# vishnutez/dps-ttc

Hardware: AMD Instinct MI355X
Metric: particles×denoise-steps/sec @256×256 N=64; x0_hat rel-L2 vs ref (higher is better)
Workload: dtype f32; 1 GPU; FFHQ-shaped 256x256 Gaussian deblur (sigma=3.0, k=61), 'ps' scale 0.3, one global best-of-N select at the end, N=64 particles (64 per GPU), t cycling 999->0; operator=gaussian_blur, step=dps, particles_per_gpu=64, global_particles=64, image=3x256x256, chains_per_gpu=3, x0_hat_store=False, semantic_stand_in=False

## Files before the change

dps_ttc_amd/csrc/api.hip:

```cpp
#include <cmath>
#include <cstring>
#include <new>
#include <algorithm>
#include <vector>

#include "common.h"

using namespace dpsx;

namespace dpsx {
static thread_local char g_hip_err[256] = "";
void set_last_hip_error(hipError_t e)
{
    snprintf(g_hip_err, sizeof(g_hip_err), "%s: %s", hipGetErrorName(e), hipGetErrorString(e));
}
}

#pragma GCC visibility push(default)
extern "C" {

int dpsx_abi_version(void) { return DPSX_ABI_VERSION; }

const char *dpsx_strerror(int code)
{
// ... 325 lines not shown
    }
    return DPSX_EUNSUPPORTED;
}

int dpsx_residual_norm_f32(const float *y, int64_t y_n, const float *ax, float *r, float *norm, int64_t n,
                           int64_t m, void *workspace, int64_t workspace_bytes, void *stream)
{
    if (!y || !ax || !norm || n < 0 || m < 0 || !rows_ok(y_n, n)) return DPSX_EINVAL;
    if (n == 0) return DPSX_OK;
    const int parts = (int)std::min<int64_t>(256, std::max<int64_t>(1, (m + 4095) / 4096));
    if (!workspace || workspace_bytes < n * parts * 4) return DPSX_EWORKSPACE;
    float *partials = static_cast<float *>(workspace);
    hipStream_t s = (hipStream_t)stream;
    int rc = residual_partials(y, y_n, ax, r, partials, n, m, parts, s);
    if (rc != DPSX_OK) return rc;
    return finalize_norm(partials, parts, norm, n, s);
}

int dpsx_norm_bwd_f32(const float *r, const float *norm, const float *g_norm, int power, float *g_ax, int64_t n,
                      int64_t m, void *stream)
{
    if (!r || !norm || !g_norm || !g_ax || n < 0 || m < 0 || (power != 1 && power != 2)) return DPSX_EINVAL;
    return norm_bwd(r, norm, g_norm, power, g_ax, n, m, (hipStream_t)stream);
}

int64_t dpsx_step_resid_bytes(const dpsx_op *op, int64_t n, int64_t c, int64_t h, int64_t w)
{
    if (!op) return DPSX_EINVAL;
    const int64_t m = meas_elems(op, c, h, w);
    if (m < 0) return DPSX_EINVAL;
    switch (op->kind) {
    case OP_MASK: return 256;
    case OP_PHASE: return phase_step_resid_bytes(op, n * c);
    default: return align256(n * m * 4);
    }
}

static bool mask_fused_ok(const dpsx_op *op, int64_t c, int64_t h, int64_t w,
                          std::initializer_list<const void *> ptrs)
{
    return (h * w) % 4 == 0 && aligned16(op->mask.mask) && vec_ok(c * h * w, ptrs);
}

int dpsx_step_draws_in_kernel(const dpsx_op *op, int64_t c, int64_t h, int64_t w)
{
    if (!op || c < 1 || h < 1 || w < 1) return 0;
    switch (op->kind) {
    case OP_IDENT: return 1;
    case OP_MASK: return (h * w) % 4 == 0 && (c * h * w) % 4 == 0;
    case OP_SEP:
    case OP_TAPS: return blur_step_draws_in_kernel(op, h, w) ? 1 : 0;
    case OP_RESIZE: return h == op->resize->in_h && w == op->resize->in_w && resize_step_draws_in_kernel(op) ? 1 : 0;
    default: return 0;
    }
}

static int step_fwd_impl(dpsx_op *op, const float *x_t, const float *model_out, const float *noise, const dpsx_rng *rng,
                         const float *y, int64_t y_n, float *x0_hat, float *sample, uint8_t *inside, void *resid,
                         float *norm, int64_t n, int64_t c, int64_t h, int64_t w, const dpsx_coefs *coefs_host,
                         void *workspace, int64_t workspace_bytes, void *stream)
{
    int rc = check_geom(op, n, c, h, w);
    if (rc != DPSX_OK) return rc;
    RngK rk{};
    if (rng) {
        if ((rc = to_rngk(rng, n, rk)) != DPSX_OK) return rc;
        if (!dpsx_step_draws_in_kernel(op, c, h, w)) return DPSX_EUNSUPPORTED;
    }
    if (!x_t || !model_out || !y || !sample || !inside || !resid || !coefs_host) return DPSX_EINVAL;
    if (!x0_hat && op && op->kind != OP_SEP && op->kind != OP_TAPS && op->kind != OP_RESIZE &&
        !(op->kind == OP_PHASE && phase_is_spectral(op)))
        return DPSX_EINVAL;
    if ((coefs_host->add_noise & 1) && !noise && !rng) return DPSX_EINVAL;
    if (!rows_ok(y_n, n)) return DPSX_EINVAL;
    if (n == 0) return DPSX_OK;
    Ws ws;
    if ((rc = carve(op, workspace, workspace_bytes, n, c, h, w, ws)) != DPSX_OK) return rc;
    hipStream_t s = (hipStream_t)stream;
    const Coefs k = to_coefs(coefs_host);
    const int64_t chw = c * h * w;
    StepFwdArgs a{x_t, model_out, noise, y, y_n, x0_hat, sample, inside, static_cast<float *>(resid),
                  ws.partials, n, c, h, w, k};
    a.y_div = row_div(y_n, n);
    a.mask_div = row_div(op->mask.rows, n);
    a.use_rng = rng != nullptr;
    a.rng = rk;
    const int parts = step_parts(op, c, h, w);
    bool tail_done = false;
    if (norm && op->d_counters && n <= kTailMaxParticles && op->kind != OP_PHASE) {
        a.tail.counters = op->d_counters;
        a.tail.partials = ws.partials;
        a.tail.parts = parts;
        a.tail.out = norm;
        tail_done = true;
    }
    switch (op->kind) {
    case OP_SEP:
    case OP_TAPS: rc = blur_step_fwd(op, a, s); break;
    case OP_RESIZE: rc = resize_step_fwd(op, a, s); break;
    case OP_MASK:
        if (!mask_fused_ok(op, c, h, w, {x_t, model_out, noise, y, x0_hat, sample}) ||
            !aligned4(inside))
            return DPSX_EUNSUPPORTED;
        rc = mask_step_fwd(op, a, parts, s);
        break;
    case OP_IDENT:
        rc = posterior_fwd(x_t, model_out, noise, a.use_rng, rk, x0_hat, sample, inside, n, chw, k, s);
        if (rc != DPSX_OK) return rc;
        rc = residual_partials(y, y_n, x0_hat, static_cast<float *>(resid), ws.partials, n, chw, parts, s, 0, nullptr, 0, 1,
                               a.tail);
        break;
    case OP_PHASE:
        rc = phase_step_fwd(op, a, static_cast<float *>(resid), s);
        break;
    default: return DPSX_EUNSUPPORTED;
    }
    if (rc != DPSX_OK) {
        if (tail_done)
            (void)hipMemsetAsync(op->d_counters, 0, kNormCounterBytes, s);
        return rc;
    }
    return (norm && !tail_done) ? finalize_norm(ws.partials, parts, norm, n, s) : DPSX_OK;
}

int dpsx_step_fwd_f32(dpsx_op *op, const float *x_t, const float *model_out, const float *noise, const float *y,
                      int64_t y_n, float *x0_hat, float *sample, uint8_t *inside, void *resid, float *norm,
                      int64_t n, int64_t c, int64_t h, int64_t w, const dpsx_coefs *coefs_host, void *workspace,
                      int64_t workspace_bytes, void *stream)
{
    return step_fwd_impl(op, x_t, model_out, noise, nullptr, y, y_n, x0_hat, sample, inside, resid, norm, n, c, h, w,
                         coefs_host, workspace, workspace_bytes, stream);
}

int dpsx_step_fwd_rng_f32(dpsx_op *op, const float *x_t, const float *model_out, const dpsx_rng *rng_host,
                          const float *y, int64_t y_n, float *x0_hat, float *sample, uint8_t *inside, void *resid,
                          float *norm, int64_t n, int64_t c, int64_t h, int64_t w, const dpsx_coefs *coefs_host,
                          void *workspace, int64_t workspace_bytes, void *stream)
{
    if (!rng_host) return DPSX_EINVAL;
    return step_fwd_impl(op, x_t, model_out, nullptr, rng_host, y, y_n, x0_hat, sample, inside, resid, norm, n, c, h, w,
                         coefs_host, workspace, workspace_bytes, stream);
}

int dpsx_step_bwd_f32(dpsx_op *op, const void *resid, const float *norm, float *norm_out, const uint8_t *inside,
                      const float *x0_hat, const float *y, int64_t y_n, float scale, int power,
                      float *g_model_out, int64_t n, int64_t c, int64_t h, int64_t w,
                      const dpsx_coefs *coefs_host, void *workspace, int64_t workspace_bytes, void *stream)
{
    return dpsx_step_bwd_extra_f32(op, resid, norm, norm_out, inside, x0_hat, y, y_n, scale, power, nullptr,
                                   g_model_out, n, c, h, w, coefs_host, workspace, workspace_bytes, stream);
}

int dpsx_step_bwd_extra_f32(dpsx_op *op, const void *resid, const float *norm, float *norm_out,
                            const uint8_t *inside, const float *x0_hat, const float *y, int64_t y_n, float scale,
                            int power, const float *g_x0_extra, float *g_model_out, int64_t n, int64_t c, int64_t h,
                            int64_t w, const dpsx_coefs *coefs_host, void *workspace, int64_t workspace_bytes,
                            void *stream)
{
    int rc = check_geom(op, n, c, h, w);
    if (rc != DPSX_OK) return rc;
    if (!resid || !inside || !g_model_out || !coefs_host || (power != 1 && power != 2)) return DPSX_EINVAL;
    if (!norm && !norm_out) return DPSX_EINVAL;
    if (y && !rows_ok(y_n, n)) return DPSX_EINVAL;
    if (n == 0) return DPSX_OK;
    Ws ws;
    if ((rc = carve(op, workspace, workspace_bytes, n, c, h, w, ws)) != DPSX_OK) return rc;
    hipStream_t s = (hipStream_t)stream;
    const Coefs k = to_coefs(coefs_host);
    const int64_t chw = c * h * w;
    const int parts = step_parts(op, c, h, w);
    if (op->kind == OP_IDENT || op->kind == OP_PHASE) {
        if (!norm && !(op->kind == OP_PHASE && phase_norm_in_bwd(op))) {
            if ((rc = finalize_norm(ws.partials, parts, norm_out, n, s)) != DPSX_OK) return rc;
            norm = norm_out;
        }
    }
    StepBwdArgs b{static_cast<const float *>(resid), norm, ws.partials, parts, norm_out, inside, x0_hat, y, y_n,
                  scale, power, g_model_out, n, c, h, w, k, g_x0_extra};
    b.y_div = row_div(y_n, n);
    b.mask_div = row_div(op->mask.rows, n);
    switch (op->kind) {
    case OP_SEP:
    case OP_TAPS: return blur_step_bwd(op, b, static_cast<float *>(ws.priv), ws.priv_bytes, s);
    case OP_RESIZE: return resize_step_bwd(op, b, s);
    case OP_MASK:
        if (!x0_hat || !y || !rows_ok(y_n, n)) return DPSX_EINVAL;
        if (!mask_fused_ok(op, c, h, w, {x0_hat, y, g_model_out}) || !aligned4(inside))
            return DPSX_EUNSUPPORTED;
        return mask_step_bwd(op, b, s);
    case OP_IDENT:
        return clamp_scale_to_eps(static_cast<const float *>(resid), norm, inside, scale, power, g_model_out, n,
                                  chw, k, s, g_x0_extra);
    case OP_PHASE:
        if (phase_vec4_ok(op) && vec_ok(h, {g_model_out, g_x0_extra}) && aligned4(inside))
            return phase_step_bwd_fused(op, const_cast<float *>(static_cast<const float *>(resid)), b, s);
        if (phase_is_spectral(op)) return DPSX_EUNSUPPORTED;
        rc = phase_step_bwd(op, const_cast<float *>(static_cast<const float *>(resid)), ws.img, n * c, s);
        if (rc != DPSX_OK) return rc;
        return clamp_scale_to_eps(ws.img, norm, inside, scale, power, g_model_out, n, chw, k, s, g_x0_extra);
    }
    return DPSX_EUNSUPPORTED;
}

int dpsx_step_update_f32(const float *sample, const float *g_model_out, const float *g_unet, float *x_next,
                         int64_t n, int64_t chw, const dpsx_coefs *coefs_host, void *stream)
{
    if (!sample || !g_model_out || !x_next || !coefs_host || n < 0 || chw < 0) return DPSX_EINVAL;
    if (coefs_host->b == 0.0f) return DPSX_EINVAL;
    return step_update(sample, g_model_out, g_unet, x_next, n, chw, to_coefs(coefs_host), (hipStream_t)stream);
}

int dpsx_corr_slots(int64_t chw) { return chw < 0 ? DPSX_EINVAL : cg_slots(chw); }

// ... 593 lines not shown
```

dps_ttc_amd/csrc/blur.hip:

```cpp
#include <algorithm>
#include <cmath>
#include <cstdlib>
#include <new>
#include <type_traits>

#include "common.h"

namespace dpsx {

constexpr int TH = 64, TW = 64, NT = 256;
constexpr size_t kScratchBytes = 1024;

struct BlurArgs {
    const float *x;
    float *out;
    const float *x_t, *model_out, *noise;
    float *x0_hat, *sample;
    uint8_t *inside_w;
    const float *y;
    unsigned y_div;
    float *partials;
    const float *norm_in;
    const float *norm_partials;
    int norm_parts;
    float *norm_out;
    const uint8_t *inside_r;
    const float *g_extra;
    float *g_model_out;
    float scale;
    int power;
    int c, h, w, tiles_x, tiles_y, planes;
    Coefs k;
    const TapRun *runs;
    int nrun[4];
    int nhlo[4], nhhi[4];
    int dbg;
    int src_h, src_w, src_off;
    int l1;
    NormTail tail;
    RngK rng;
};

__device__ __forceinline__ bool block_to_tile(const BlurArgs &a, int &plane, int &ty, int &tx)
{
    const int tiles = a.tiles_x * a.tiles_y;
    const int b = blockIdx.x;
    const int xcd = b & 7, k = b >> 3;
    plane = (k / tiles) * 8 + xcd;
    const int t = k % tiles;
    ty = t / a.tiles_x;
    tx = t % a.tiles_x;
    return plane < a.planes;
}

__device__ __forceinline__ int clampi(int v, int lo, int hi) { return v < lo ? lo : (v > hi ? hi : v); }

template <bool POST, bool REFLECT, bool VEC>
__device__ __forceinline__ void load_region(float *s_in, const int SW, const int RH, const int RW,
                                            const int gy0, const int gx0, const int h0, const int w0,
                                            const BlurArgs &a, const int plane, const int tid = threadIdx.x)
{
    const int h = REFLECT ? a.h : a.src_h, w = REFLECT ? a.w : a.src_w, off = REFLECT ? 0 : a.src_off;
    const int64_t hw = (int64_t)h * w;
    const int n = plane / a.c, ch = plane % a.c;
    const float *src = nullptr, *eps = nullptr, *vv = nullptr, *zz = nullptr;
    if constexpr (POST) {
        src = a.x_t + (int64_t)plane * hw;
        eps = a.model_out + ((int64_t)n * 2 * a.c + ch) * hw;
        vv = eps + (int64_t)a.c * hw;
        zz = a.noise + (int64_t)plane * hw;
    } else {
        src = a.x + (int64_t)plane * hw;
    }
// ... 1093 lines not shown

static inline unsigned grid_blocks(const BlurArgs &a)
{
    const int groups = (a.planes + 7) / 8;
    return (unsigned)(groups * 8 * a.tiles_x * a.tiles_y);
}

int64_t blur_parts_per_particle(const dpsx_op *, int64_t c, int64_t h, int64_t w)
{
    return c * ((h + TH - 1) / TH) * ((w + TW - 1) / TW);
}

template <auto Kernel, class... Args>
static int launch(const BlurArgs &a, size_t lds, hipStream_t s, const Args &...args)
{
    return launch_lds<Kernel>(grid_blocks(a), NT, lds, s, a, args...);
}

template <class F> static int with_r4(int r4, F &&f)
{
    switch (r4) {
    case 1: return f(std::integral_constant<int, 1>{});
    case 2: return f(std::integral_constant<int, 2>{});
    case 3: return f(std::integral_constant<int, 3>{});
    case 4: return f(std::integral_constant<int, 4>{});
    case 5: return f(std::integral_constant<int, 5>{});
    case 6: return f(std::integral_constant<int, 6>{});
    case 7: return f(std::integral_constant<int, 7>{});
    case 8: return f(std::integral_constant<int, 8>{});
    }
    return DPSX_EUNSUPPORTED;
}

template <bool POST, bool RESID, bool RNG = false>
static int dispatch_sep_fwd(const BlurTables &b, const BlurArgs &a, hipStream_t s)
{
    return with_r4(b.radius4 / 4, [&](auto r4) {
        constexpr int R4 = decltype(r4)::value;
        return launch<k_blur_sep_fwd<R4, POST, RESID, RNG>>(a, sep_lds_bytes(4 * R4), s, b.sep);
    });
}

template <int R4, bool EPI>
static int launch_sep_adj(const BlurArgs &a, const SepTaps &t, int reach, hipStream_t s)
{
    const size_t lds = sep_lds_bytes(4 * R4, a.h % TH == 0 && a.w % TW == 0 && a.tiles_x >= 2 && a.tiles_y >= 2);
    if constexpr (EPI) {
        if (a.g_extra) return launch<k_blur_sep_adj<R4, true, true>>(a, lds, s, t, reach);
    }
    return launch<k_blur_sep_adj<R4, EPI, false>>(a, lds, s, t, reach);
}

template <int R4, bool EPI>
static int launch_sep_adj_sym(const BlurArgs &a, const SepTaps &t, hipStream_t s)
{
    const size_t lds = sep_lds_bytes(4 * R4, true);
    if constexpr (EPI) {
        if (a.g_extra) return launch<k_blur_sep_adj_sym<R4, true, true>>(a, lds, s, t);
    }
    return launch<k_blur_sep_adj_sym<R4, EPI, false>>(a, lds, s, t);
}

static bool sep_adj_sym_ok(const BlurTables &b, const BlurArgs &a)
{
    static const char *force = getenv("DPSX_SEP_ADJ");
    if (force && force[0] == 'f') return false;
    const int rr = b.radius4;
    if (a.h % TH != 0 || a.w % TW != 0 || a.tiles_x < 2 || a.tiles_y < 2 || rr + 1 >= a.h || rr + 1 >= a.w) return false;
    for (int i = 0; i < rr; ++i)
        if (b.sep.h[i] != b.sep.h[2 * rr - i] || b.sep.v[i] != b.sep.v[2 * rr - i]) return false;
    return true;
}

template <bool EPI>
static int dispatch_sep_adj(const BlurTables &b, const BlurArgs &a, hipStream_t s)
{
    const int rr = b.radius4;
    const bool sym = sep_adj_sym_ok(b, a);
    SepTaps f{};
    if (!sym)
        for (int i = 0; i <= 2 * rr; ++i) {
            f.h[i] = b.sep.h[2 * rr - i];
            f.v[i] = b.sep.v[2 * rr - i];
        }
    return with_r4(rr / 4, [&](auto r4) {
        constexpr int R4 = decltype(r4)::value;
        return sym ? launch_sep_adj_sym<R4, EPI>(a, b.sep, s) : launch_sep_adj<R4, EPI>(a, f, b.reach, s);
    });
}

// ... 132 lines not shown
int blur_forward(const dpsx_op *op, const float *x, float *y, int64_t planes, int64_t h, int64_t w, hipStream_t s)
{
    if (!geometry_ok(op, h, w)) return DPSX_EINVAL;
    if (planes == 0) return DPSX_OK;
    BlurArgs a{};
    a.x = x; a.out = y;
    fill_geometry(a, planes, 1, h, w);
    const bool vec = blur_vec(h, w, {x, y});
    return op->kind == OP_SEP && vec ? dispatch_sep_fwd<false, false>(op->blur->t, a, s)
                                     : launch_taps_fwd<false, false>(*op->blur, a, vec, s);
}

int blur_adjoint(const dpsx_op *op, const float *u, float *g, int64_t planes, int64_t h, int64_t w, float *scratch,
                 int64_t scratch_bytes, hipStream_t s)
{
    if (!geometry_ok(op, h, w)) return DPSX_EINVAL;
    if (planes == 0) return DPSX_OK;
    BlurArgs a{};
    a.x = u; a.out = g;
    fill_geometry(a, planes, 1, h, w);
    const bool vec = blur_vec(h, w, {u, g});
    return op->kind == OP_SEP && vec ? dispatch_sep_adj<false>(op->blur->t, a, s)
                                     : launch_taps_adj<false>(*op->blur, a, vec, scratch, scratch_bytes, s);
}

bool blur_step_draws_in_kernel(const dpsx_op *op, int64_t h, int64_t w)
{
    if (!geometry_ok(op, h, w) || h % TH != 0 || w % TW != 0) return false;
    const BlurTables &b = op->blur->t;
    if (op->kind == OP_SEP) return b.radius4 < h && b.radius4 < w && b.radius4 / 4 >= 1 && b.radius4 / 4 <= 8;
    return std::max(b.halo_t, b.halo_b) < h && std::max(b.halo_l, b.halo_r) < w;
}

int blur_step_fwd(const dpsx_op *op, const StepFwdArgs &f, hipStream_t s)
{
    if (!geometry_ok(op, f.h, f.w)) return DPSX_EINVAL;
    if (f.n == 0) return DPSX_OK;
    BlurArgs a{};
    a.x_t = f.x_t; a.model_out = f.model_out; a.noise = f.noise;
    a.x0_hat = f.x0_hat; a.sample = f.sample; a.inside_w = f.inside;
    a.y = f.y; a.y_div = f.y_div; a.out = f.resid; a.partials = f.partials;
    a.k = f.k;
    fill_geometry(a, f.n * f.c, f.c, f.h, f.w);
    a.tail = f.tail;
    a.tail.blocks_per_particle = a.c * a.tiles_x * a.tiles_y;
    const bool vec = blur_vec(f.h, f.w, {f.x_t, f.model_out, f.noise, f.x0_hat, f.sample, f.y, f.resid}) && aligned4(f.inside);
    if (f.use_rng) {
        if (!vec || !blur_step_draws_in_kernel(op, f.h, f.w)) return DPSX_EUNSUPPORTED;
        a.rng = f.rng;
        return op->kind == OP_SEP ? dispatch_sep_fwd<true, true, true>(op->blur->t, a, s)
                                  : launch_taps_fwd<true, true, true>(*op->blur, a, true, s);
    }
    return op->kind == OP_SEP && vec ? dispatch_sep_fwd<true, true>(op->blur->t, a, s)
                                     : launch_taps_fwd<true, true>(*op->blur, a, vec, s);
}

int blur_step_bwd(const dpsx_op *op, const StepBwdArgs &b, float *scratch, int64_t scratch_bytes, hipStream_t s)
{
    if (!geometry_ok(op, b.h, b.w)) return DPSX_EINVAL;
    if (b.n == 0) return DPSX_OK;
    BlurArgs a{};
    a.x = b.resid;
    a.norm_in = b.norm; a.norm_partials = b.partials; a.norm_parts = b.parts; a.norm_out = b.norm_out;
    a.inside_r = b.inside; a.g_extra = b.g_extra; a.g_model_out = b.g_model_out; a.scale = b.scale; a.power = b.power;
    a.k = b.k;
    fill_geometry(a, b.n * b.c, b.c, b.h, b.w);
    const bool vec = blur_vec(b.h, b.w, {b.resid, b.g_model_out, b.g_extra}) && aligned4(b.inside);
    return op->kind == OP_SEP && vec ? dispatch_sep_adj<true>(op->blur->t, a, s)
                                     : launch_taps_adj<true>(*op->blur, a, vec, scratch, scratch_bytes, s);
}

int blur_score(const dpsx_op *op, const float *x, const float *y, int64_t y_n, float *partials, int64_t n,
               int64_t c, int64_t h, int64_t w, int l1, hipStream_t s)
{
    if (!geometry_ok(op, h, w)) return DPSX_EINVAL;
    if (n == 0) return DPSX_OK;
    BlurArgs a{};
    a.x = x; a.y = y; a.y_div = row_div(y_n, n); a.out = nullptr; a.partials = partials;
    fill_geometry(a, n * c, c, h, w);
    a.l1 = l1;
    const bool vec = blur_vec(h, w, {x, y});
    return op->kind == OP_SEP && vec ? dispatch_sep_fwd<false, true>(op->blur->t, a, s)
                                     : launch_taps_fwd<false, true>(*op->blur, a, vec, s);
}

}
```

dps_ttc_amd/csrc/blur_sep.h:

```cpp

__device__ __forceinline__ int fold_sources(int i, int n, int R, int (&p)[2])
{
    int cnt = 0;
    p[0] = p[1] = 0;
    if (i >= 1 && i <= R) p[cnt++] = -i;
    if (i <= n - 2 && i >= n - 1 - R) p[cnt++] = 2 * (n - 1) - i;
    return cnt;
}

#ifndef DPSX_ABLATION
#define DPSX_ABLATION 0
#endif
#define ABL(bit) (DPSX_ABLATION && (a.dbg & (bit)))

typedef float v2f __attribute__((ext_vector_type(2)));
typedef float v4f __attribute__((ext_vector_type(4)));

__device__ __forceinline__ float4 ld_stream(const float *p, bool nt)
{
    if (nt) {
        const v4f v = __builtin_nontemporal_load(reinterpret_cast<const v4f *>(p));
        return make_float4(v.x, v.y, v.z, v.w);
    }
    return *reinterpret_cast<const float4 *>(p);
}
__device__ __forceinline__ void st_stream(float *p, const float4 &v, bool nt)
{
    if (nt) __builtin_nontemporal_store(v4f{v.x, v.y, v.z, v.w}, reinterpret_cast<v4f *>(p));
    else *reinterpret_cast<float4 *>(p) = v;
}

__device__ __forceinline__ int sep_slot()
{
    const int t = threadIdx.x, l5 = t & 31, q = l5 >> 2;
    const int grp = 2 * ((t >> 5) & 1) + (__popc(q) & 1), pos = 4 * (q >> 1) + (l5 & 3);
    return (t & ~63) | (16 * grp + pos);
}

template <int RR>
struct SepGeom {
    static constexpr int RH = TH + 2 * RR;
    static constexpr int RW = TW + 2 * RR;
    static constexpr int SW = RW + 4;
    static constexpr int RWU = RW / 4;
    static constexpr int HALO_TB = RR * RWU;
    static constexpr int HALO_LR = TH * (RR / 4);
    static constexpr int HALO = 2 * HALO_TB + 2 * HALO_LR;
    static constexpr int HALO_PER_THREAD = (HALO + NT - 1) / NT;
    static constexpr int FOLD_PER_THREAD = (RH * 2 * RR + NT - 1) / NT;
};

template <int RR>
__device__ __forceinline__ void halo_unit(int hu, int &rr, int &cu)
{
    using G = SepGeom<RR>;
    constexpr int Q = RR / 4;
    const unsigned t = (unsigned)hu, v = (unsigned)max(hu - 2 * G::HALO_TB, 0);
    const unsigned r_tb = t / G::RWU, c_tb = t - r_tb * G::RWU;
    const unsigned r_lr = v / (2 * Q), c_lr = v - r_lr * (2 * Q);
    const bool tb = hu < 2 * G::HALO_TB;
    rr = tb ? (int)(r_tb < RR ? r_tb : r_tb + TH) : (int)r_lr + RR;
    cu = tb ? (int)c_tb : (int)(c_lr < Q ? c_lr : c_lr + (TW / 4));
}

template <int D>
constexpr bool small_div_exact()
{
    for (unsigned n = 0; n < 4096; ++n)
        if (((n * (((1u << 20) + D - 1) / D)) >> 20) != n / D) return false;
    return true;
// ... 210 lines not shown
{
    const bool outx = unit_mirrored(gx, w), outy = gy < 0 || gy >= h;
    int sy, sx;
    if constexpr (REFLECT) {
        sy = gy < 0 ? -gy : (gy >= h ? 2 * (h - 1) - gy : gy);
        sx = gx < 0 ? -gx - 3 : (gx >= w ? 2 * w - 5 - gx : gx);
    } else {
        sy = clampi(gy, 0, h - 1);
        sx = clampi(gx, 0, w - 4);
    }
    const float *p = plane + (unsigned)(sy * w + sx);
    if constexpr (!REFLECT) p = (outx || outy) ? g_zero_unit : p;
    const v4fu v = *reinterpret_cast<const v4fu *>(p);
    return make_float4(v.x, v.y, v.z, v.w);
}

__device__ __forceinline__ float4 unit_unmirror(const float4 &u, bool mirrored)
{
    float x = u.x, y = u.y, z = u.z, w = u.w;
    asm volatile("" : "+v"(x), "+v"(y), "+v"(z), "+v"(w));
    return make_float4(mirrored ? w : x, mirrored ? z : y, mirrored ? y : z, mirrored ? x : w);
}

template <bool REFLECT>
__device__ __forceinline__ float4 load_unit_reg(const float *plane, int gy, int gx, int h, int w)
{
    const float4 v = load_unit_raw<REFLECT>(plane, gy, gx, h, w);
    if constexpr (REFLECT) return unit_mirrored(gx, w) ? make_float4(v.w, v.z, v.y, v.x) : v;
    else return v;
}

template <int RR, bool POST, bool REFLECT, bool RNG = false>
__device__ __forceinline__ void load_region_reg(float *s, const int h0, const int w0, const BlurArgs &a,
                                                const int plane)
{
    using G = SepGeom<RR>;
    const int h = a.h, w = a.w;
    const unsigned hw = (unsigned)(h * w);
    const int n = plane / a.c, ch = plane % a.c;
    const float *src, *eps = nullptr, *vv = nullptr, *zz = nullptr;
    if constexpr (POST) {
        src = a.x_t + (int64_t)plane * hw;
        eps = a.model_out + ((int64_t)n * 2 * a.c + ch) * hw;
        vv = eps + (int64_t)a.c * hw;
        if constexpr (!RNG) zz = a.noise + (int64_t)plane * hw;
    } else {
        src = a.x + (int64_t)plane * hw;
    }
    constexpr int NI = TH * TW / 4 / NT;
    constexpr int NH = G::HALO_PER_THREAD;
    float4 xi[NI], ei[NI], vi[NI], zi[NI], xh[NH], eh[NH];
    int hrr[NH], hcu[NH];
    halo_units_deal<RR>(threadIdx.x, hrr, hcu);
    int tid = threadIdx.x;
    if constexpr (POST) asm volatile("" : "+v"(tid));
#pragma unroll
    for (int pass = 0; pass < (POST ? 2 : 1); ++pass) {
        const float *p = pass ? eps : src;
#pragma unroll
        for (int k = 0; k < NI; ++k) {
            const int u = threadIdx.x + k * NT, row = u >> 4, cu = u & 15;
            const float4 v = *reinterpret_cast<const float4 *>(p + (unsigned)((h0 + row) * w + w0 + 4 * cu));
            if (pass) ei[k] = v; else xi[k] = v;
        }
#pragma unroll
        for (int k = 0; k < NH; ++k) {
            const float4 v = load_unit_raw<REFLECT || POST>(p, h0 - RR + hrr[k], w0 - RR + 4 * hcu[k], h, w);
// ... 5 lines not shown
#pragma unroll
            for (int k = 0; k < NI; ++k) {
                const int u = threadIdx.x + k * NT, row = u >> 4, cu = u & 15;
                const unsigned o = (unsigned)((h0 + row) * w + w0 + 4 * cu);
                vi[k] = ld_stream(vv + o, true);
                if constexpr (!RNG) zi[k] = ld_stream(zz + o, true);
            }
        } else {
#pragma unroll
            for (int k = 0; k < NI; ++k) vi[k] = zi[k] = make_float4(0, 0, 0, 0);
        }
    }
    __builtin_amdgcn_sched_barrier(0);
#pragma unroll
    for (int k = 0; k < NI; ++k) {
        const int u = threadIdx.x + k * NT, row = u >> 4, cu = u & 15;
        float4 val = xi[k];
        if constexpr (POST) {
            float4 x0, sm;
            uchar4 gate;
            float4 zk = make_float4(0, 0, 0, 0);
            if constexpr (RNG) {
                if (a.k.add_noise & 1)
                    zk = rng_unit(a.rng, ((unsigned)ch * hw + (unsigned)((h0 + row) * w + w0 + 4 * cu)) >> 2,
                                  rng_particle(a.rng, (unsigned)n));
            } else {
                zk = zi[k];
            }
            post_unit(xi[k], ei[k], vi[k], zk, a.k, x0, sm, gate);
            const int64_t o = (int64_t)plane * hw + (unsigned)((h0 + row) * w + w0 + 4 * cu);
            if (a.x0_hat) *reinterpret_cast<float4 *>(a.x0_hat + o) = x0;
            *reinterpret_cast<float4 *>(a.sample + o) = sm;
            *reinterpret_cast<uchar4 *>(a.inside_w + o) = gate;
            val = x0;
        }
        *reinterpret_cast<float4 *>(s + (RR + row) * G::SW + RR + 4 * cu) = val;
    }
    if constexpr (POST) halo_units_deal<RR>(tid, hrr, hcu);
#pragma unroll
    for (int k = 0; k < NH; ++k) {
        if (k * NT + NT > G::HALO && (int)threadIdx.x + k * NT >= G::HALO) continue;
        float4 val = xh[k];
        if constexpr (POST) val = post_x0_unit(xh[k], eh[k], a.k);
        if constexpr (REFLECT || POST) val = unit_unmirror(val, unit_mirrored(w0 - RR + 4 * hcu[k], w));
        *reinterpret_cast<float4 *>(s + hrr[k] * G::SW + 4 * hcu[k]) = val;
    }
}

template <int RR, int FOLD = 0>
__device__ __forceinline__ void hpass_inplace(float *s, const float (&taps)[2 * kMaxRadius + 1])
{
    using G = SepGeom<RR>;
    constexpr int NG = TW / 8, NF = (8 + 2 * RR) / 4, WN = 8 + 2 * RR;
    for (int it = sep_slot(); it < G::RH * NG; it += NT) {
        const int rr = it / NG, g = it - rr * NG;
        float *row = s + rr * G::SW + g * 8;
        float win[WN];
#pragma unroll
        for (int j = 0; j < NF; ++j) {
            const float4 v = *reinterpret_cast<const float4 *>(row + 4 * j);
            win[4 * j] = v.x; win[4 * j + 1] = v.y; win[4 * j + 2] = v.z; win[4 * j + 3] = v.w;
        }
        v2f acc2[4];
#pragma unroll
        for (int p = 0; p < 4; ++p) acc2[p] = v2f{0.0f, 0.0f};
#pragma unroll
// ... 99 lines not shown
                }
        }
    }
    if constexpr (FOLD == 2) {
        if (rg >= (TH - 1 - RR) / 4) {
#pragma unroll
            for (int RG = (TH - 1 - RR) / 4; RG < TH / 4; ++RG)
                if (rg == RG) {
#pragma unroll
                    for (int m = 0; m < RR; ++m) {
                        const float4 v4 = *reinterpret_cast<const float4 *>(s + (TH - 1 - m + RR) * G::SW + 4 * cg);
#pragma unroll
                        for (int i = 0; i < 4; ++i) {
                            const int jb = TH - 1 - (4 * RG + i);
                            if (jb >= 1 && jb <= RR && m <= RR - jb) {
                                acc[i][0] = fmaf(taps[RR - jb - m], v4.x, acc[i][0]);
                                acc[i][1] = fmaf(taps[RR - jb - m], v4.y, acc[i][1]);
                                acc[i][2] = fmaf(taps[RR - jb - m], v4.z, acc[i][2]);
                                acc[i][3] = fmaf(taps[RR - jb - m], v4.w, acc[i][3]);
                            }
                        }
                    }
                }
        }
    }
}

constexpr int sep_waves_per_simd(int r4, bool light = false)
{
    return light ? (r4 <= 3 ? 4 : (r4 <= 7 ? 2 : 1)) : (r4 <= 3 ? 4 : (r4 <= 5 ? 3 : 2));
}
constexpr int sep_adj_waves_per_simd(int r4) { return r4 <= 6 ? sep_waves_per_simd(r4) : 1; }

template <bool EXTRA>
__device__ __forceinline__ void adj_gate_epilogue(const BlurArgs &a, const int plane, const unsigned o, const float (&acc)[4][4],
                                                  const uchar4 (&gate)[4], const float coef)
{
    const unsigned hw = (unsigned)(a.h * a.w);
    const int n = plane / a.c, ch = plane % a.c;
    float *gp = a.g_model_out + ((int64_t)n * 2 * a.c + ch) * hw + o;
    const v2f mb2{-a.k.b, -a.k.b}, c2{coef, coef};
    float4 ex[4];
#pragma unroll
    for (int i = 0; i < 4; ++i) ex[i] = make_float4(0, 0, 0, 0);
    if constexpr (EXTRA) {
        const float *ep = a.g_extra + (int64_t)plane * hw + o;
#pragma unroll
        for (int i = 0; i < 4; ++i) ex[i] = *reinterpret_cast<const float4 *>(ep + (unsigned)(i * a.w));
    }
#pragma unroll
    for (int i = 0; i < 4; ++i) {
        const v2f lo = mb2 * (c2 * v2f{acc[i][0], acc[i][1]} + v2f{ex[i].x, ex[i].y});
        const v2f hi = mb2 * (c2 * v2f{acc[i][2], acc[i][3]} + v2f{ex[i].z, ex[i].w});
        float4 g;
        g.x = gate[i].x ? lo.x : 0.0f;
        g.y = gate[i].y ? lo.y : 0.0f;
        g.z = gate[i].z ? hi.x : 0.0f;
        g.w = gate[i].w ? hi.y : 0.0f;
        *reinterpret_cast<float4 *>(gp + (unsigned)(i * a.w)) = g;
    }
}

template <int R4, bool POST, bool RESID, bool RNG = false>
__global__ __launch_bounds__(NT, sep_waves_per_simd(R4, !POST && !RESID)) void k_blur_sep_fwd(BlurArgs a, SepTaps taps)
{
    constexpr int RR = 4 * R4;
    using G = SepGeom<RR>;
    extern __shared__ __align__(16) float lds[];
    float *s = lds, *s_red = lds + G::RH * G::SW;
    int plane, ty, tx;
    if (!block_to_tile(a, plane, ty, tx)) return;
    const int h0 = ty * TH, w0 = tx * TW;
    const bool regular = a.h % TH == 0 && a.w % TW == 0 && RR < a.h && RR < a.w && !ABL(128);
    if constexpr (RNG) load_region_reg<RR, POST, true, true>(s, h0, w0, a, plane);
    else if (regular) load_region_reg<RR, POST, true>(s, h0, w0, a, plane);
    else if (!ABL(4)) load_region_fast<RR, POST, true>(s, h0, w0, a, plane);
    else for (int i = threadIdx.x; i < G::RH * G::SW; i += NT) s[i] = (float)i;
    const int slot = sep_slot(), cg = slot & 15, rg = slot >> 4;
    const int ox = w0 + 4 * cg;
    __syncthreads();
    if (!ABL(1)) hpass_inplace<RR>(s, taps.h);
    __syncthreads();
    float acc[4][4];
    if (!ABL(2)) vpass_regs<RR>(s, acc, rg, cg, taps.v);
    else for (int i = 0; i < 4; ++i) for (int e = 0; e < 4; ++e) acc[i][e] = s[(4 * rg + i + RR) * G::SW + 4 * cg + e];
    float ss = 0.0f;
    if (RESID && regular) {
        if (!ABL(8)) {
            const unsigned hw = (unsigned)(a.h * a.w), o = (unsigned)((h0 + 4 * rg) * a.w + ox);
            const int n = plane / a.c, ch = plane % a.c;
            const float *yp = a.y + ((int64_t)meas_row((unsigned)n, a.y_div) * a.c + ch) * hw + o;
            float *rp = a.out ? a.out + (int64_t)plane * hw + o : nullptr;
            float4 yv[4];
#pragma unroll
            for (int i = 0; i < 4; ++i) yv[i] = *reinterpret_cast<const float4 *>(yp + (unsigned)(i * a.w));
#pragma unroll
            for (int i = 0; i < 4; ++i) {
                float4 r;
                r.x = yv[i].x - acc[i][0]; r.y = yv[i].y - acc[i][1]; r.z = yv[i].z - acc[i][2]; r.w = yv[i].w - acc[i][3];
                if (rp) *reinterpret_cast<float4 *>(rp + (unsigned)(i * a.w)) = r;
                if constexpr (POST) ss += r.x * r.x + r.y * r.y + r.z * r.z + r.w * r.w;
                else ss += a.l1 ? fabsf(r.x) + fabsf(r.y) + fabsf(r.z) + fabsf(r.w)
                                : r.x * r.x + r.y * r.y + r.z * r.z + r.w * r.w;
            }
        }
    } else if (ox < a.w && !ABL(8)) {
#pragma unroll
        for (int i = 0; i < 4; ++i) {
            const int oy = h0 + 4 * rg + i;
            if constexpr (RESID) ss += resid_epilogue<true>(a, plane, oy, ox, acc[i]);
            else out_epilogue<true>(a, plane, oy, ox, acc[i], 0.0f, false);
        }
    }
    if constexpr (RESID) {
        const float t = block_sum(ss, s_red);
        if (threadIdx.x == 0) tail_publish(&a.partials[(int64_t)plane * (a.tiles_x * a.tiles_y) + ty * a.tiles_x + tx], t, POST && a.tail.counters != nullptr);
        if constexpr (POST) tail_arrive(a.tail, plane / a.c);
    }
}


template <int R4, bool EPI, bool EXTRA = false>
__global__ __launch_bounds__(NT, sep_adj_waves_per_simd(R4)) void k_blur_sep_adj(BlurArgs a, SepTaps taps, int reach)
{
    constexpr int RR = 4 * R4;
    using G = SepGeom<RR>;
    extern __shared__ __align__(16) float lds[];
    float *s = lds, *s_nrm = lds + G::RH * G::SW, *s_th = s_nrm + 4, *s_tv = s_th + 80;
    int plane, ty, tx;
    if (!block_to_tile(a, plane, ty, tx)) return;
    const int h0 = ty * TH, w0 = tx * TW;
    float coef = 0.0f;
    const bool regular = a.h % TH == 0 && a.w % TW == 0 && !ABL(128);
    const bool norm_split = EPI && !a.norm_in && regular && a.norm_parts <= 4 * kWave;
    NormPartials np;
    if constexpr (EPI) {
        if (norm_split) np = particle_norm_issue(a.norm_partials, a.norm_parts, plane / a.c);
        else if (!a.norm_in) particle_norm_to_lds(a.norm_partials, a.norm_parts, plane / a.c, s_nrm);
// ... 80 lines not shown
#pragma unroll
        for (int i = 0; i < 4; ++i) {
            const int oy = h0 + 4 * rg + i;
            if (oy >= a.h) continue;
            if (oy >= 1 && oy <= reach) {
                for (int m = 0; m <= reach - oy; ++m) {
                    const int row = m - (h0 - RR);
                    if (row < 0 || row >= G::RH) continue;
                    const float4 v4 = *reinterpret_cast<const float4 *>(s + row * G::SW + 4 * cg);
                    const float t = s_tv[RR + oy + m];
                    acc[i][0] = fmaf(t, v4.x, acc[i][0]);
                    acc[i][1] = fmaf(t, v4.y, acc[i][1]);
                    acc[i][2] = fmaf(t, v4.z, acc[i][2]);
                    acc[i][3] = fmaf(t, v4.w, acc[i][3]);
                }
            }
            const int jb = a.h - 1 - oy;
            if (jb >= 1 && jb <= reach) {
                for (int m = 0; m <= reach - jb; ++m) {
                    const int row = (a.h - 1 - m) - (h0 - RR);
                    if (row < 0 || row >= G::RH) continue;
                    const float4 v4 = *reinterpret_cast<const float4 *>(s + row * G::SW + 4 * cg);
                    const float t = s_tv[RR - jb - m];
                    acc[i][0] = fmaf(t, v4.x, acc[i][0]);
                    acc[i][1] = fmaf(t, v4.y, acc[i][1]);
                    acc[i][2] = fmaf(t, v4.z, acc[i][2]);
                    acc[i][3] = fmaf(t, v4.w, acc[i][3]);
                }
            }
        }
    }
    const int ox = w0 + 4 * cg;
    if (EPI && regular) {
        if (!ABL(8)) adj_gate_epilogue<EXTRA>(a, plane, (unsigned)((h0 + 4 * rg) * a.w + ox), acc, gate, coef);
    } else if (ox < a.w && !ABL(8)) {
#pragma unroll
        for (int i = 0; i < 4; ++i) out_epilogue<true>(a, plane, h0 + 4 * rg + i, ox, acc[i], coef, EPI);
    }
}

template <int R4, bool EPI, bool EXTRA = false>
__global__ __launch_bounds__(NT, sep_adj_waves_per_simd(R4)) void k_blur_sep_adj_sym(BlurArgs a, SepTaps taps)
{
    constexpr int RR = 4 * R4;
    using G = SepGeom<RR>;
    extern __shared__ __align__(16) float lds[];
    float *s = lds, *s_nrm = lds + G::RH * G::SW;
    int plane, ty, tx;
    if (!block_to_tile(a, plane, ty, tx)) return;
    const int h0 = ty * TH, w0 = tx * TW;
    float coef = 0.0f;
    const bool norm_split = EPI && !a.norm_in && a.norm_parts <= 4 * kWave;
    NormPartials np;
    if constexpr (EPI) {
        if (norm_split) np = particle_norm_issue(a.norm_partials, a.norm_parts, plane / a.c);
        else if (!a.norm_in) particle_norm_to_lds(a.norm_partials, a.norm_parts, plane / a.c, s_nrm);
    }
    const int slot = sep_slot(), cg = slot & 15, rg = slot >> 4;
    uchar4 gate[4];
    if constexpr (EPI) {
        const uint8_t *ip = a.inside_r + (int64_t)plane * a.h * a.w + (unsigned)((h0 + 4 * rg) * a.w + w0 + 4 * cg);
#pragma unroll
        for (int i = 0; i < 4; ++i) gate[i] = *reinterpret_cast<const uchar4 *>(ip + (unsigned)(i * a.w));
    }
    load_region_reg<RR, false, true>(s, h0, w0, a, plane);
    if constexpr (EPI) { if (norm_split) particle_norm_reduce(np, a.norm_parts, s_nrm); }
    __syncthreads();
    if constexpr (EPI) {
        const float nv = a.norm_in ? a.norm_in[plane / a.c] : s_nrm[0];
        coef = norm_coef_dev(nv, a.scale, a.power);
        if (!a.norm_in && a.norm_out && threadIdx.x == 0 && ty == 0 && tx == 0 && plane % a.c == 0)
            a.norm_out[plane / a.c] = nv;
    }
    const int br = h0 == 0 ? RR : (h0 + TH == a.h ? RR + TH - 1 : -1);
    const int bc = w0 == 0 ? RR : (w0 + TW == a.w ? RR + TW - 1 : -1);
    if (br >= 0 || bc >= 0) {
        const int t = threadIdx.x;
        if (br >= 0 && t < G::RW) s[br * G::SW + t] *= (t == bc ? 4.0f : 2.0f);
        if (bc >= 0 && t >= NT / 2 && t - NT / 2 < G::RH && t - NT / 2 != br) s[(t - NT / 2) * G::SW + bc] *= 2.0f;
        __syncthreads();
    }
    hpass_inplace<RR, 0>(s, taps.h);
    __syncthreads();
    float acc[4][4];
    vpass_regs<RR, 0>(s, acc, rg, cg, taps.v);
    const int ox = w0 + 4 * cg, oy = h0 + 4 * rg;
    if (br >= 0 || bc >= 0) {
#pragma unroll
        for (int i = 0; i < 4; ++i) {
            const float fy = (oy + i == 0 || oy + i == a.h - 1) ? 0.5f : 1.0f;
#pragma unroll
            for (int e = 0; e < 4; ++e) acc[i][e] *= ((ox + e == 0 || ox + e == a.w - 1) ? 0.5f : 1.0f) * fy;
        }
    }
    if constexpr (EPI) {
        adj_gate_epilogue<EXTRA>(a, plane, (unsigned)(oy * a.w + ox), acc, gate, coef);
    } else {
#pragma unroll
        for (int i = 0; i < 4; ++i) out_epilogue<true>(a, plane, oy + i, ox, acc[i], coef, false);
    }
}
```

dps_ttc_amd/csrc/common.h:

```cpp
#pragma once
#include <hip/hip_runtime.h>
#include <initializer_list>
#include <stdint.h>
#include <stdio.h>
#include <vector>

#include "../../include/dpsx.h"

namespace dpsx {

constexpr int kWave = 64;

void set_last_hip_error(hipError_t e);

inline int check_launch()
{
    hipError_t e = hipGetLastError();
    if (e != hipSuccess) {
        set_last_hip_error(e);
        return DPSX_ELAUNCH;
    }
    return DPSX_OK;
}

// ... 374 lines not shown
    int nrun[4] = {0, 0, 0, 0};
    int nrun_adj_pos[4] = {0, 0, 0, 0}, nrun_adj_neg[4] = {0, 0, 0, 0};
    int halo_t = 0, halo_b = 0, halo_l = 0, halo_r = 0;
};

struct BlurOp {
    BlurTables t;
    const TapRun *d_runs_fwd = nullptr, *d_runs_adj = nullptr;
    DeviceTables tables;
};

struct ResizeOp {
    int64_t in_h = 0, in_w = 0, out_h = 0, out_w = 0, taps_h = 0, taps_w = 0;
};

struct PhaseOp {
    int64_t h = 0, pad = 0, planes = 0;
};

struct MaskOp {
    const float *mask = nullptr;
    int64_t rows = 1, h = 0, w = 0;
};

}

struct dpsx_op {
    int kind = OP_IDENT;
    dpsx::BlurOp *blur = nullptr;
    dpsx::ResizeOp *resize = nullptr;
    dpsx::PhaseOp *phase = nullptr;
    dpsx::MaskOp mask{};
    unsigned *d_counters = nullptr;
};

namespace dpsx {

struct StepFwdArgs {
    const float *x_t, *model_out, *noise, *y;
    int64_t y_n;
    float *x0_hat, *sample;
    uint8_t *inside;
    float *resid;
    float *partials;
    int64_t n, c, h, w;
    Coefs k;
    NormTail tail{};
    unsigned y_div = 0, mask_div = 0;
    bool use_rng = false;
    RngK rng{};
};

struct StepBwdArgs {
    const float *resid, *norm;
    const float *partials;
    int parts;
    float *norm_out;
    const uint8_t *inside;
    const float *x0_hat, *y;
    int64_t y_n;
    float scale;
    int power;
    float *g_model_out;
    int64_t n, c, h, w;
    Coefs k;
    const float *g_extra = nullptr;
    unsigned y_div = 0, mask_div = 0;
};

BlurTables blur_tables(const float *kernel_host, int ks, int mode);
int blur_create(dpsx_op *op, const float *kernel_host, int ks, int mode);
void blur_destroy(dpsx_op *op);
int blur_forward(const dpsx_op *op, const float *x, float *y, int64_t planes, int64_t h, int64_t w, hipStream_t s);
int blur_adjoint(const dpsx_op *op, const float *u, float *g, int64_t planes, int64_t h, int64_t w, float *scratch,
                 int64_t scratch_bytes, hipStream_t s);
int64_t blur_adjoint_scratch_bytes(const dpsx_op *op, int64_t planes, int64_t h, int64_t w);
int blur_step_fwd(const dpsx_op *op, const StepFwdArgs &a, hipStream_t s);
bool blur_step_draws_in_kernel(const dpsx_op *op, int64_t h, int64_t w);
int blur_step_bwd(const dpsx_op *op, const StepBwdArgs &a, float *scratch, int64_t scratch_bytes, hipStream_t s);
int blur_score(const dpsx_op *op, const float *x, const float *y, int64_t y_n, float *partials,
               int64_t n, int64_t c, int64_t h, int64_t w, int l1, hipStream_t s);
int64_t blur_parts_per_particle(const dpsx_op *op, int64_t c, int64_t h, int64_t w);


int resize_create(dpsx_op *op, const ResizeOp &shape, const float *w_h, const int64_t *i_h, const float *w_w,
                  const int64_t *i_w);
void resize_destroy(dpsx_op *op);
int64_t resize_parts_per_particle(const dpsx_op *op, int64_t c);
int resize_forward(const dpsx_op *op, const float *x, float *y, int64_t planes, hipStream_t s);
int resize_adjoint(const dpsx_op *op, const float *u, float *g, int64_t planes, hipStream_t s);
int resize_step_fwd(const dpsx_op *op, const StepFwdArgs &a, hipStream_t s);
bool resize_step_draws_in_kernel(const dpsx_op *op);
int resize_step_bwd(const dpsx_op *op, const StepBwdArgs &a, hipStream_t s);
int resize_score(const dpsx_op *op, const float *x, const float *y, int64_t y_n, float *partials,
                 int64_t n, int64_t c, int l1, hipStream_t s);

int posterior_fwd(const float *x, const float *mo, const float *z, bool use_rng, const RngK &r, float *x0, float *sample,
                  uint8_t *inside, int64_t n, int64_t chw, const Coefs &k, hipStream_t s, bool one_state = false,
                  int64_t states = 1);
int randn_f32(float *out, uint32_t *bits, int64_t n, int64_t chw, const RngK &r, hipStream_t s);
int posterior_bwd(const float *g_x0, const float *g_s, const float *x, const float *mo, const float *z,
                  float *g_x, float *g_mo, int64_t n, int64_t chw, const Coefs &k, hipStream_t s);
int mask_mul(const float *x, const float *mask, float *y, int64_t planes, int64_t hw, hipStream_t s, int64_t c = 1,
             unsigned mask_div = 0);
int residual_partials(const float *y, int64_t y_n, const float *ax, float *r, float *partials,
                      int64_t n, int64_t m, int parts, hipStream_t s, int l1 = 0, const float *mask = nullptr,
                      int64_t hw = 0, int64_t mask_n = 1, const NormTail &tail = NormTail{});
int finalize_norm(const float *partials, int parts, float *norm, int64_t n, hipStream_t s);
int finalize_select(const CostArgs &t, int segments, hipStream_t s);
int finalize_select_copy(const CostArgs &t, int segments, const float *src, float *dst, int64_t chw, hipStream_t s);
// ... 97 lines not shown
```

Baseline: 590,600 particle-steps/s.

## Pass clamp gate as per-wave ballot bitmasks from blur forward to adjoint

The fused separable-blur forward step now packs the per-pixel clamp gate (inside flags) into 64-bit per-wave ballot masks. It stages the flags in LDS and stores the masks in an extension of the residual buffer. The adjoint epilogue loads these masks with scalar loads and uses inverse ballot in place of re-reading the byte-per-pixel inside array from global memory. The aim is to cut the backward pass's global traffic for the gate from one byte per pixel to one bit. The cost is extra LDS and ballot work in the forward kernel, a larger residual allocation, and a stamp check on the op to make sure the masks match the current call.

```diff
diff --git a/dps_ttc_amd/csrc/api.hip b/dps_ttc_amd/csrc/api.hip
--- a/dps_ttc_amd/csrc/api.hip
+++ b/dps_ttc_amd/csrc/api.hip
@@ -381,8 +381,16 @@
     switch (op->kind) {
     case OP_MASK: return 256;
     case OP_PHASE: return phase_step_resid_bytes(op, n * c);
+    case OP_SEP: return align256(n * m * 4) + blur_gate_mask_bytes(op, n, c, h, w);
     default: return align256(n * m * 4);
     }
+}
+
+static unsigned long long *gate_masks_at(const dpsx_op *op, const void *resid, int64_t n, int64_t c, int64_t h, int64_t w)
+{
+    if (op->kind != OP_SEP || blur_gate_mask_bytes(op, n, c, h, w) == 0) return nullptr;
+    auto *base = const_cast<unsigned char *>(static_cast<const unsigned char *>(resid));
+    return reinterpret_cast<unsigned long long *>(base + align256(n * c * h * w * 4));
 }
 
 static bool mask_fused_ok(const dpsx_op *op, int64_t c, int64_t h, int64_t w,
@@ -443,9 +451,12 @@
         a.tail.out = norm;
         tail_done = true;
     }
+    op->gate_stamp = dpsx_op::GateStamp{};
+    bool masks_written = false;
+    a.gate_masks = gate_masks_at(op, resid, n, c, h, w);
     switch (op->kind) {
     case OP_SEP:
-    case OP_TAPS: rc = blur_step_fwd(op, a, s); break;
+    case OP_TAPS: rc = blur_step_fwd(op, a, s, &masks_written); break;
     case OP_RESIZE: rc = resize_step_fwd(op, a, s); break;
     case OP_MASK:
         if (!mask_fused_ok(op, c, h, w, {x_t, model_out, noise, y, x0_hat, sample}) ||
@@ -469,6 +480,7 @@
             (void)hipMemsetAsync(op->d_counters, 0, kNormCounterBytes, s);
         return rc;
     }
+    if (masks_written) op->gate_stamp = dpsx_op::GateStamp{resid, inside, n, c, h, w};
     return (norm && !tail_done) ? finalize_norm(ws.partials, parts, norm, n, s) : DPSX_OK;
 }
 
@@ -528,6 +540,9 @@
                   scale, power, g_model_out, n, c, h, w, k, g_x0_extra};
     b.y_div = row_div(y_n, n);
     b.mask_div = row_div(op->mask.rows, n);
+    const dpsx_op::GateStamp &st = op->gate_stamp;
+    if (st.resid && st.resid == resid && st.inside == inside && st.n == n && st.c == c && st.h == h && st.w == w)
+        b.gate_masks = gate_masks_at(op, resid, n, c, h, w);
     switch (op->kind) {
     case OP_SEP:
     case OP_TAPS: return blur_step_bwd(op, b, static_cast<float *>(ws.priv), ws.priv_bytes, s);
diff --git a/dps_ttc_amd/csrc/blur.hip b/dps_ttc_amd/csrc/blur.hip
--- a/dps_ttc_amd/csrc/blur.hip
+++ b/dps_ttc_amd/csrc/blur.hip
@@ -10,6 +10,8 @@
 
 constexpr int TH = 64, TW = 64, NT = 256;
 constexpr size_t kScratchBytes = 1024;
+constexpr size_t kGateLdsBytes = TH * TW;
+constexpr int kGateMaskTileBytes = (NT / 64) * 16 * 8;
 
 struct BlurArgs {
     const float *x;
@@ -39,6 +41,7 @@
     int l1;
     NormTail tail;
     RngK rng;
+    unsigned long long *gate_masks;
 };
 
 __device__ __forceinline__ bool block_to_tile(const BlurArgs &a, int &plane, int &ty, int &tx)
@@ -1198,12 +1201,24 @@
     return DPSX_EUNSUPPORTED;
 }
 
+static bool sep_gate_masks_ok(const BlurTables &b, int64_t h, int64_t w)
+{
+    return h % TH == 0 && w % TW == 0 && b.radius4 < h && b.radius4 < w && b.radius4 / 4 >= 1 && b.radius4 / 4 <= 8;
+}
+
+int64_t blur_gate_mask_bytes(const dpsx_op *op, int64_t n, int64_t c, int64_t h, int64_t w)
+{
+    if (op->kind != OP_SEP || !sep_gate_masks_ok(op->blur->t, h, w)) return 0;
+    return n * c * (h / TH) * (w / TW) * kGateMaskTileBytes;
+}
+
 template <bool POST, bool RESID, bool RNG = false>
 static int dispatch_sep_fwd(const BlurTables &b, const BlurArgs &a, hipStream_t s)
 {
     return with_r4(b.radius4 / 4, [&](auto r4) {
         constexpr int R4 = decltype(r4)::value;
-        return launch<k_blur_sep_fwd<R4, POST, RESID, RNG>>(a, sep_lds_bytes(4 * R4), s, b.sep);
+        const size_t lds = sep_lds_bytes(4 * R4) + (POST ? kGateLdsBytes : 0);
+        return launch<k_blur_sep_fwd<R4, POST, RESID, RNG>>(a, lds, s, b.sep);
     });
 }
 
@@ -1222,6 +1237,9 @@
 {
     const size_t lds = sep_lds_bytes(4 * R4, true);
     if constexpr (EPI) {
+        if (a.gate_masks)
+            return a.g_extra ? launch<k_blur_sep_adj_sym<R4, true, true, true>>(a, lds, s, t)
+                             : launch<k_blur_sep_adj_sym<R4, true, false, true>>(a, lds, s, t);
         if (a.g_extra) return launch<k_blur_sep_adj_sym<R4, true, true>>(a, lds, s, t);
     }
     return launch<k_blur_sep_adj_sym<R4, EPI, false>>(a, lds, s, t);
@@ -1420,8 +1438,9 @@
     return std::max(b.halo_t, b.halo_b) < h && std::max(b.halo_l, b.halo_r) < w;
 }
 
-int blur_step_fwd(const dpsx_op *op, const StepFwdArgs &f, hipStream_t s)
-{
+int blur_step_fwd(const dpsx_op *op, const StepFwdArgs &f, hipStream_t s, bool *masks_written)
+{
+    if (masks_written) *masks_written = false;
     if (!geometry_ok(op, f.h, f.w)) return DPSX_EINVAL;
     if (f.n == 0) return DPSX_OK;
     BlurArgs a{};
@@ -1433,14 +1452,20 @@
     a.tail = f.tail;
     a.tail.blocks_per_particle = a.c * a.tiles_x * a.tiles_y;
     const bool vec = blur_vec(f.h, f.w, {f.x_t, f.model_out, f.noise, f.x0_hat, f.sample, f.y, f.resid}) && aligned4(f.inside);
+    if (op->kind == OP_SEP && vec && f.resid && f.gate_masks && sep_gate_masks_ok(op->blur->t, f.h, f.w))
+        a.gate_masks = f.gate_masks;
+    int rc;
     if (f.use_rng) {
         if (!vec || !blur_step_draws_in_kernel(op, f.h, f.w)) return DPSX_EUNSUPPORTED;
         a.rng = f.rng;
-        return op->kind == OP_SEP ? dispatch_sep_fwd<true, true, true>(op->blur->t, a, s)
-                                  : launch_taps_fwd<true, true, true>(*op->blur, a, true, s);
-    }
-    return op->kind == OP_SEP && vec ? dispatch_sep_fwd<true, true>(op->blur->t, a, s)
-                                     : launch_taps_fwd<true, true>(*op->blur, a, vec, s);
+        rc = op->kind == OP_SEP ? dispatch_sep_fwd<true, true, true>(op->blur->t, a, s)
+                                : launch_taps_fwd<true, true, true>(*op->blur, a, true, s);
+    } else {
+        rc = op->kind == OP_SEP && vec ? dispatch_sep_fwd<true, true>(op->blur->t, a, s)
+                                       : launch_taps_fwd<true, true>(*op->blur, a, vec, s);
+    }
+    if (masks_written) *masks_written = rc == DPSX_OK && a.gate_masks != nullptr;
+    return rc;
 }
 
 int blur_step_bwd(const dpsx_op *op, const StepBwdArgs &b, float *scratch, int64_t scratch_bytes, hipStream_t s)
@@ -1454,6 +1479,7 @@
     a.k = b.k;
     fill_geometry(a, b.n * b.c, b.c, b.h, b.w);
     const bool vec = blur_vec(b.h, b.w, {b.resid, b.g_model_out, b.g_extra}) && aligned4(b.inside);
+    if (op->kind == OP_SEP && vec) a.gate_masks = const_cast<unsigned long long *>(b.gate_masks);
     return op->kind == OP_SEP && vec ? dispatch_sep_adj<true>(op->blur->t, a, s)
                                      : launch_taps_adj<true>(*op->blur, a, vec, scratch, scratch_bytes, s);
 }
diff --git a/dps_ttc_amd/csrc/blur_sep.h b/dps_ttc_amd/csrc/blur_sep.h
--- a/dps_ttc_amd/csrc/blur_sep.h
+++ b/dps_ttc_amd/csrc/blur_sep.h
@@ -36,6 +36,8 @@
     const int grp = 2 * ((t >> 5) & 1) + (__popc(q) & 1), pos = 4 * (q >> 1) + (l5 & 3);
     return (t & ~63) | (16 * grp + pos);
 }
+
+__device__ __forceinline__ int gate_lds_word(int row, int cu) { return (((row >> 2) * (TW / 4) + cu) << 2) + (row & 3); }
 
 template <int RR>
 struct SepGeom {
@@ -312,7 +314,7 @@
 
 template <int RR, bool POST, bool REFLECT, bool RNG = false>
 __device__ __forceinline__ void load_region_reg(float *s, const int h0, const int w0, const BlurArgs &a,
-                                                const int plane)
+                                                const int plane, uint8_t *s_gate = nullptr)
 {
     using G = SepGeom<RR>;
     const int h = a.h, w = a.w;
@@ -384,6 +386,7 @@
             if (a.x0_hat) *reinterpret_cast<float4 *>(a.x0_hat + o) = x0;
             *reinterpret_cast<float4 *>(a.sample + o) = sm;
             *reinterpret_cast<uchar4 *>(a.inside_w + o) = gate;
+            *reinterpret_cast<uchar4 *>(s_gate + 4 * gate_lds_word(row, cu)) = gate;
             val = x0;
         }
         *reinterpret_cast<float4 *>(s + (RR + row) * G::SW + RR + 4 * cu) = val;
@@ -549,9 +552,44 @@
 }
 constexpr int sep_adj_waves_per_simd(int r4) { return r4 <= 6 ? sep_waves_per_simd(r4) : 1; }
 
-template <bool EXTRA>
+struct GateMasks {
+    unsigned long long m[16];
+};
+
+__device__ __forceinline__ int64_t gate_mask_index(const BlurArgs &a, int plane, int ty, int tx, int wave)
+{
+    return ((((int64_t)plane * a.tiles_y + ty) * a.tiles_x + tx) * (NT / 64) + wave) * 16;
+}
+
+__device__ __forceinline__ void gate_masks_store(const BlurArgs &a, const uint8_t *s_gate, int plane, int ty, int tx,
+                                                 int rg, int cg)
+{
+    const uint4 gb = *reinterpret_cast<const uint4 *>(s_gate + 16 * (rg * (TW / 4) + cg));
+    const unsigned wd[4] = {gb.x, gb.y, gb.z, gb.w};
+    const int lane = threadIdx.x & 63;
+    unsigned long long mine = 0;
+#pragma unroll
+    for (int i = 0; i < 4; ++i)
+#pragma unroll
+        for (int e = 0; e < 4; ++e) {
+            const unsigned long long m = __ballot((wd[i] >> (8 * e)) & 0xffu);
+            mine = lane == 4 * i + e ? m : mine;
+        }
+    if (lane < 16) a.gate_masks[gate_mask_index(a, plane, ty, tx, threadIdx.x >> 6) + lane] = mine;
+}
+
+__device__ __forceinline__ void gate_masks_load(const BlurArgs &a, int plane, int ty, int tx, GateMasks &gm)
+{
+    typedef const unsigned long long __attribute__((address_space(4))) *const_masks;
+    const int wave = __builtin_amdgcn_readfirstlane(threadIdx.x >> 6);
+    const const_masks p = (const_masks)(a.gate_masks + gate_mask_index(a, plane, ty, tx, wave));
+#pragma unroll
+    for (int j = 0; j < 16; ++j) gm.m[j] = p[j];
+}
+
+template <bool EXTRA, bool MASKS = false>
 __device__ __forceinline__ void adj_gate_epilogue(const BlurArgs &a, const int plane, const unsigned o, const float (&acc)[4][4],
-                                                  const uchar4 (&gate)[4], const float coef)
+                                                  const uchar4 (&gate)[4], const float coef, const GateMasks &gm)
 {
     const unsigned hw = (unsigned)(a.h * a.w);
     const int n = plane / a.c, ch = plane % a.c;
@@ -570,10 +608,17 @@
         const v2f lo = mb2 * (c2 * v2f{acc[i][0], acc[i][1]} + v2f{ex[i].x, ex[i].y});
         const v2f hi = mb2 * (c2 * v2f{acc[i][2], acc[i][3]} + v2f{ex[i].z, ex[i].w});
         float4 g;
-        g.x = gate[i].x ? lo.x : 0.0f;
-        g.y = gate[i].y ? lo.y : 0.0f;
-        g.z = gate[i].z ? hi.x : 0.0f;
-        g.w = gate[i].w ? hi.y : 0.0f;
+        if constexpr (MASKS) {
+            g.x = __builtin_amdgcn_inverse_ballot_w64(gm.m[4 * i]) ? lo.x : 0.0f;
+            g.y = __builtin_amdgcn_inverse_ballot_w64(gm.m[4 * i + 1]) ? lo.y : 0.0f;
+            g.z = __builtin_amdgcn_inverse_ballot_w64(gm.m[4 * i + 2]) ? hi.x : 0.0f;
+            g.w = __builtin_amdgcn_inverse_ballot_w64(gm.m[4 * i + 3]) ? hi.y : 0.0f;
+        } else {
+            g.x = gate[i].x ? lo.x : 0.0f;
+            g.y = gate[i].y ? lo.y : 0.0f;
+            g.z = gate[i].z ? hi.x : 0.0f;
+            g.w = gate[i].w ? hi.y : 0.0f;
+        }
         *reinterpret_cast<float4 *>(gp + (unsigned)(i * a.w)) = g;
     }
 }
@@ -585,12 +630,13 @@
     using G = SepGeom<RR>;
     extern __shared__ __align__(16) float lds[];
     float *s = lds, *s_red = lds + G::RH * G::SW;
+    uint8_t *s_gate = reinterpret_cast<uint8_t *>(s_red) + kScratchBytes;
     int plane, ty, tx;
     if (!block_to_tile(a, plane, ty, tx)) return;
     const int h0 = ty * TH, w0 = tx * TW;
     const bool regular = a.h % TH == 0 && a.w % TW == 0 && RR < a.h && RR < a.w && !ABL(128);
-    if constexpr (RNG) load_region_reg<RR, POST, true, true>(s, h0, w0, a, plane);
-    else if (regular) load_region_reg<RR, POST, true>(s, h0, w0, a, plane);
+    if constexpr (RNG) load_region_reg<RR, POST, true, true>(s, h0, w0, a, plane, s_gate);
+    else if (regular) load_region_reg<RR, POST, true>(s, h0, w0, a, plane, s_gate);
     else if (!ABL(4)) load_region_fast<RR, POST, true>(s, h0, w0, a, plane);
     else for (int i = threadIdx.x; i < G::RH * G::SW; i += NT) s[i] = (float)i;
     const int slot = sep_slot(), cg = slot & 15, rg = slot >> 4;
@@ -621,6 +667,7 @@
                                 : r.x * r.x + r.y * r.y + r.z * r.z + r.w * r.w;
             }
         }
+        if constexpr (POST) { if (a.gate_masks) gate_masks_store(a, s_gate, plane, ty, tx, rg, cg); }
     } else if (ox < a.w && !ABL(8)) {
 #pragma unroll
         for (int i = 0; i < 4; ++i) {
@@ -767,14 +814,14 @@
     }
     const int ox = w0 + 4 * cg;
     if (EPI && regular) {
-        if (!ABL(8)) adj_gate_epilogue<EXTRA>(a, plane, (unsigned)((h0 + 4 * rg) * a.w + ox), acc, gate, coef);
+        if (!ABL(8)) adj_gate_epilogue<EXTRA>(a, plane, (unsigned)((h0 + 4 * rg) * a.w + ox), acc, gate, coef, GateMasks{});
     } else if (ox < a.w && !ABL(8)) {
 #pragma unroll
         for (int i = 0; i < 4; ++i) out_epilogue<true>(a, plane, h0 + 4 * rg + i, ox, acc[i], coef, EPI);
     }
 }
 
-template <int R4, bool EPI, bool EXTRA = false>
+template <int R4, bool EPI, bool EXTRA = false, bool MASKS = false>
 __global__ __launch_bounds__(NT, sep_adj_waves_per_simd(R4)) void k_blur_sep_adj_sym(BlurArgs a, SepTaps taps)
 {
     constexpr int RR = 4 * R4;
@@ -793,7 +840,7 @@
     }
     const int slot = sep_slot(), cg = slot & 15, rg = slot >> 4;
     uchar4 gate[4];
-    if constexpr (EPI) {
+    if constexpr (EPI && !MASKS) {
         const uint8_t *ip = a.inside_r + (int64_t)plane * a.h * a.w + (unsigned)((h0 + 4 * rg) * a.w + w0 + 4 * cg);
 #pragma unroll
         for (int i = 0; i < 4; ++i) gate[i] = *reinterpret_cast<const uchar4 *>(ip + (unsigned)(i * a.w));
@@ -817,6 +864,8 @@
     }
     hpass_inplace<RR, 0>(s, taps.h);
     __syncthreads();
+    GateMasks gm;
+    if constexpr (MASKS) gate_masks_load(a, plane, ty, tx, gm);
     float acc[4][4];
     vpass_regs<RR, 0>(s, acc, rg, cg, taps.v);
     const int ox = w0 + 4 * cg, oy = h0 + 4 * rg;
@@ -829,7 +878,7 @@
         }
     }
     if constexpr (EPI) {
-        adj_gate_epilogue<EXTRA>(a, plane, (unsigned)(oy * a.w + ox), acc, gate, coef);
+        adj_gate_epilogue<EXTRA, MASKS>(a, plane, (unsigned)(oy * a.w + ox), acc, gate, coef, gm);
     } else {
 #pragma unroll
         for (int i = 0; i < 4; ++i) out_epilogue<true>(a, plane, oy + i, ox, acc[i], coef, false);
diff --git a/dps_ttc_amd/csrc/common.h b/dps_ttc_amd/csrc/common.h
--- a/dps_ttc_amd/csrc/common.h
+++ b/dps_ttc_amd/csrc/common.h
@@ -430,6 +430,11 @@
     dpsx::PhaseOp *phase = nullptr;
     dpsx::MaskOp mask{};
     unsigned *d_counters = nullptr;
+    struct GateStamp {
+        const void *resid = nullptr;
+        const uint8_t *inside = nullptr;
+        int64_t n = 0, c = 0, h = 0, w = 0;
+    } gate_stamp;
 };
 
 namespace dpsx {
@@ -447,6 +452,7 @@
     unsigned y_div = 0, mask_div = 0;
     bool use_rng = false;
     RngK rng{};
+    unsigned long long *gate_masks = nullptr;
 };
 
 struct StepBwdArgs {
@@ -464,6 +470,7 @@
     Coefs k;
     const float *g_extra = nullptr;
     unsigned y_div = 0, mask_div = 0;
+    const unsigned long long *gate_masks = nullptr;
 };
 
 BlurTables blur_tables(const float *kernel_host, int ks, int mode);
@@ -473,7 +480,8 @@
 int blur_adjoint(const dpsx_op *op, const float *u, float *g, int64_t planes, int64_t h, int64_t w, float *scratch,
                  int64_t scratch_bytes, hipStream_t s);
 int64_t blur_adjoint_scratch_bytes(const dpsx_op *op, int64_t planes, int64_t h, int64_t w);
-int blur_step_fwd(const dpsx_op *op, const StepFwdArgs &a, hipStream_t s);
+int blur_step_fwd(const dpsx_op *op, const StepFwdArgs &a, hipStream_t s, bool *masks_written = nullptr);
+int64_t blur_gate_mask_bytes(const dpsx_op *op, int64_t n, int64_t c, int64_t h, int64_t w);
 bool blur_step_draws_in_kernel(const dpsx_op *op, int64_t h, int64_t w);
 int blur_step_bwd(const dpsx_op *op, const StepBwdArgs &a, float *scratch, int64_t scratch_bytes, hipStream_t s);
 int blur_score(const dpsx_op *op, const float *x, const float *y, int64_t y_n, float *partials,
```

Result: slower. 583,900 particle-steps/s (-1.1%).
